# asmuth-archive/libsmatrix

Measured on NVIDIA B200. Metric: incr_mops_c2, higher is better.
Workload: dtype u32

## Files before the change

libsmatrix_b200/csrc/smx_host.c:

```c
#define _GNU_SOURCE
#include <cuda_runtime_api.h>
#include <pthread.h>
#include <stdarg.h>
#include <stdio.h>
#include <stdlib.h>
#include <string.h>
#include <time.h>
#include <errno.h>
#include <fcntl.h>
#include <sys/stat.h>
#include <sys/types.h>
#include <unistd.h>

#include "../../include/smatrix.h"
#include "../../include/smatrix_b200.h"
#include "../../include/smatrix_batch.h"
#include "smx_internal.h"

#define SMX_DIR_LOG_DEFAULT 20u
#define SMX_CHUNK_DEFAULT (1u << 26)
#define SMX_STAGE_MAX (1u << 23)
#define SMX_SEG_MIN ((size_t)64 << 20)
#define SMX_SEG_MAX ((size_t)16 << 30)
#define SMX_MAX_ROUNDS 128
// ... 262 lines not shown
}
static void scratch_free(smatrix_t* s, void* p) {
  if (p && !s->arena_bytes) cudaFree(p);
}

static void ensure_lists(smatrix_t* s, uint32_t n) {
  if (n <= s->list_cap) return;
  uint32_t cap = s->list_cap ? s->list_cap : 1024;
  while (cap < n) cap *= 2;
  if (cap > s->chunk_max) cap = s->chunk_max > n ? s->chunk_max : n;
  if (s->arena_bytes && cap < s->chunk_max) cap = s->chunk_max;
  if (s->list_cap) {
    CK(cudaStreamSynchronize(s->stream));
    scratch_free(s, s->defer[0]); scratch_free(s, s->defer[1]); scratch_free(s, s->lists.late);
    scratch_free(s, s->lists.grow); scratch_free(s, s->lists.t0rows); scratch_free(s, s->lists.plan);
    scratch_free(s, s->lists.big); scratch_free(s, s->lists.mid);
  }
  s->defer[0] = (uint32_t*)scratch_alloc(s, (size_t)cap * 4);
  s->defer[1] = (uint32_t*)scratch_alloc(s, (size_t)cap * 4);
  s->lists.late = (uint32_t*)scratch_alloc(s, (size_t)cap * 4);
  s->lists.grow = (uint32_t*)scratch_alloc(s, (size_t)cap * 4);
  s->lists.t0rows = (uint32_t*)scratch_alloc(s, (size_t)cap * 4);
  s->lists.plan = (smx_plan_t*)scratch_alloc(s, (size_t)cap * sizeof(smx_plan_t));
  s->lists.big = (uint32_t*)scratch_alloc(s, (size_t)cap * 4);
  s->lists.mid = (uint32_t*)scratch_alloc(s, (size_t)cap * 4);
  s->list_cap = cap;
}

static void ensure_stage(smatrix_t* s, uint32_t n) {
  if (n <= s->stage_cap) return;
  uint32_t cap = n < 4096 ? 4096 : n;
  if (s->arena_bytes && cap < s->stage_max) cap = s->stage_max;
  if (s->stage_cap) {
    CK(cudaStreamSynchronize(s->stream));
    CK(cudaStreamSynchronize(s->copy_stream));
    for (int b = 0; b < 2; b++)
      for (int a = 0; a < 3; a++) scratch_free(s, s->stage[b][a]);
  }
  for (int b = 0; b < 2; b++)
    for (int a = 0; a < 3; a++) s->stage[b][a] = (uint32_t*)scratch_alloc(s, (size_t)cap * 4);
// ... 28 lines not shown
    if (have) CK(cudaMemcpyAsync(nb, s->free_ptr[c], (size_t)have * 8, cudaMemcpyDeviceToDevice, s->stream));
    s->free_ptr[c] = nb;
    copy_h2d(s, &s->d_ctl->free_stack[c], &s->free_ptr[c], sizeof nb, s->stream);
    s->free_cap[c] = (uint32_t)cap;
  }
}

static void grow_rows(smatrix_t* s, uint32_t n_grow) {
  smx_view_t v = view_of(s);
  double t0 = now_ns();
  smx_launch_grow_plan(s->stream, v, s->lists, n_grow);
  s->n_launches++;
  read_ctl(s);
  double t1 = now_ns();
  const size_t bytes = (size_t)s->h_ctl->plan_bytes;
  const uint32_t n_big = s->h_ctl->n_big, n_mid = s->h_ctl->n_mid;
  char* region = bytes ? slab_reserve(s, bytes) : NULL;
  s->bucket_bytes += bytes;
  if (s->recycle) {
    ensure_free_stacks(s);
    smx_launch_free_push(s->stream, v, s->lists, n_grow);
    s->n_launches++;
  }
  double t2 = now_ns();
  if (bytes && s->h_ctl->need_zero) CK(cudaMemsetAsync(region, 0, bytes, s->stream));
  const int tiles = s->migrate_tiles && n_big;
  smx_launch_migrate(s->stream, v, s->lists, n_grow, n_mid, n_big, region, tiles);
  if (tiles) {
    unsigned long long* spill;
    uint32_t n_spill;
    for (;;) {
      spill = dbuf_need(s, &s->db.spill, (size_t)s->spill_cap * 16);
      CK(cudaMemsetAsync(&s->d_ctl->n_spill, 0, 4, s->stream));
      smx_launch_migrate_tiles(s->stream, v, s->lists, n_big, region, spill, s->spill_cap);
      copy_d2h(s, &s->h_small->n_spill, &s->d_ctl->n_spill, 4, s->stream);
      CK(cudaStreamSynchronize(s->stream));
      n_spill = s->h_small->n_spill;
      if (n_spill <= s->spill_cap) break;
      s->spill_cap = n_spill + n_spill / 2 + 1024;
    }
    smx_launch_migrate_tiles_finish(s->stream, v, s->lists, n_big, region, spill, n_spill);
    s->n_spilled += n_spill;
  }
  if (s->timing) CK(cudaStreamSynchronize(s->stream));
  s->n_launches += (n_grow > n_mid + n_big ? 1 : 0) + (n_mid ? 1 : 0) + (n_big ? 3 : 0);
  s->n_row_grows += n_grow;
  s->n_recycled += s->h_ctl->n_recycled;
  s->phase_ns[PH_GROW_PLAN] += t1 - t0;
  s->phase_ns[PH_SLAB] += t2 - t1;
  s->phase_ns[PH_MIGRATE] += now_ns() - t2;
}

static double ln_unit(double r) {
  int k = 0;
  while (r < 0.5) { r *= 2.0; k++; }
  const double y = (r - 1.0) / (r + 1.0), y2 = y * y;
  double term = y, sum = 0.0;
  for (int i = 1; i < 40; i += 2) { sum += term / (double)i; term *= y2; }
  return 2.0 * sum - (double)k * 0.69314718055994530942;
}
// ... 1151 lines not shown
  if (s->fname && snapshot_save(s) != 0) {
    printf("libsmatrix error: could not write %s; the previous snapshot (if any) was kept\n", s->fname);
    fflush(stdout);
  }
  for (int i = 0; i < s->nsegs; i++)
    if (s->segs[i].owned) cudaFree(s->segs[i].base);
  free(s->segs);
  if (!s->dir_in_arena) cudaFree(s->dir);
  cudaFree(s->d_ctl);
  cudaFreeHost(s->h_ctl);
  cudaFree(s->d_small);
  cudaFreeHost(s->h_small);
  if (s->list_cap) {
    scratch_free(s, s->defer[0]); scratch_free(s, s->defer[1]); scratch_free(s, s->lists.late);
    scratch_free(s, s->lists.grow); scratch_free(s, s->lists.t0rows); scratch_free(s, s->lists.plan);
    scratch_free(s, s->lists.big); scratch_free(s, s->lists.mid);
  }
  scratch_free(s, s->addrs);
  if (s->part_cap)
    for (int a = 0; a < 4; a++) scratch_free(s, s->part[a]);
  if (s->stage_cap)
    for (int b = 0; b < 2; b++)
      for (int a = 0; a < 3; a++) scratch_free(s, s->stage[b][a]);
  const smx_dbuf_t* db = (const smx_dbuf_t*)&s->db;
  for (size_t b = 0; b < sizeof s->db / sizeof *db; b++) cudaFree(db[b].p);
  cudaEventDestroy(s->stage_ready[0]); cudaEventDestroy(s->stage_ready[1]);
  cudaEventDestroy(s->ev0); cudaEventDestroy(s->ev1);
  cudaEventDestroy(s->t_start); cudaEventDestroy(s->t_stop);
  cudaStreamDestroy(s->stream);
  cudaStreamDestroy(s->copy_stream);
  cudaStreamDestroy(s->read_stream[0]); cudaStreamDestroy(s->read_stream[1]);
// ... 93 lines not shown
      break;
    case SMX_STAT_RECYCLED: r = s->n_recycled; break;
    case SMX_STAT_BUCKET_BYTES: r = s->bucket_bytes; break;
    case SMX_STAT_SPILLED: r = s->n_spilled; break;
    case SMX_STAT_SLICED_GETS: r = s->n_sliced_gets; break;
    case SMX_STAT_WIDE_CHUNKS: r = s->n_wide_chunks; break;
    case SMX_STAT_NS_ALLOC: r = (uint64_t)s->alloc_ns; break;
    case SMX_STAT_ALLOCS: r = s->n_allocs; break;
    case SMX_STAT_TOPK_BIG: r = s->n_topk_big; break;
    case SMX_STAT_TOPK_PASSES: r = s->n_topk_passes; break;
    case SMX_STAT_H2D_BYTES: r = s->h2d_bytes; break;
    case SMX_STAT_D2H_BYTES: r = s->d2h_bytes; break;
    case SMX_STAT_DIR_CAP: r = s->dir_cap; break;
    case SMX_STAT_SLAB_BYTES: r = s->slab_bytes; break;
    case SMX_STAT_DEVICE_BYTES: {
      r = s->seg_bytes + s->dir_cap * sizeof(smx_row_t) + (uint64_t)s->list_cap * (6 * 4 + sizeof(smx_plan_t)) +
          (uint64_t)s->stage_cap * 24 + (uint64_t)s->addrs_cap * 8 + (uint64_t)s->part_cap * 16;
      const smx_dbuf_t* db = (const smx_dbuf_t*)&s->db;
      for (size_t b = 0; b < sizeof s->db / sizeof *db; b++) r += db[b].bytes;
      break;
    }
    case SMX_STAT_LAUNCHES: r = s->n_launches; break;
    case SMX_STAT_ROUNDS: r = s->n_rounds; break;
    case SMX_STAT_ROW_GROWS: r = s->n_row_grows; break;
    case SMX_STAT_DIR_GROWS: r = s->n_dir_grows; break;
    case SMX_STAT_KERNEL_NS: r = (uint64_t)s->kernel_ns; break;
    case SMX_STAT_NS_PARTITION: r = (uint64_t)s->phase_ns[PH_PARTITION]; break;
    case SMX_STAT_NS_UPSERT: r = (uint64_t)s->phase_ns[PH_UPSERT]; break;
    case SMX_STAT_NS_GROW_PLAN: r = (uint64_t)s->phase_ns[PH_GROW_PLAN]; break;
    case SMX_STAT_NS_SLAB: r = (uint64_t)s->phase_ns[PH_SLAB]; break;
    case SMX_STAT_NS_MIGRATE: r = (uint64_t)s->phase_ns[PH_MIGRATE]; break;
// ... 322 lines not shown
```

libsmatrix_b200/csrc/smx_internal.h:

```cpp
#ifndef SMX_INTERNAL_H
#define SMX_INTERNAL_H

#include <stddef.h>
#include <stdint.h>

#ifdef __cplusplus
extern "C" {
#endif

#define SMX_META_CAPLOG 0x3Fu
#define SMX_META_USED   0x100u
#define SMX_META_ZC     0x200u
#define SMX_META_D      0x400u
#define SMX_META_SLOG_SHIFT 16
#define SMX_META_SLOG   (0x1Fu << SMX_META_SLOG_SHIFT)
#define SMX_META_T0P    0x800u
#define SMX_META_GROW   0x1000u
#define SMX_INLINE_LOG  2u
#define SMX_MIN_SLAB_LOG 4u
#define SMX_MAX_CAPLOG  31u
#define SMX_BIG_LOG     13u
#define SMX_MID_LOG     9u
#define SMX_ZERO_LOG    9u
#define SMX_CLASSES     32u
#define SMX_PLAN_RECYCLED (1ull << 63)

typedef struct {
  uint32_t key;
  uint32_t meta;
  uint64_t slots;
  uint32_t live;
  uint32_t c0;
  uint32_t t0inv;
  uint32_t want;
  uint64_t inl[4];
} smx_row_t;

#define SMX_DIR_SLICES 256u
#define SMX_DIR_CREATE_STEPS 256u
typedef struct {
  unsigned long long dir_used;
  uint32_t n_late;
  uint32_t n_t0;
  uint32_t n_defer;
  uint32_t n_dirfull;
  uint32_t n_grow;
  uint32_t n_big;
  uint32_t n_mid;
  uint32_t n_recycled;
  uint32_t n_spill;
  uint32_t dir_probe_max;
  unsigned long long plan_bytes;
  unsigned long long need_zero;
  uint32_t grow_from[SMX_CLASSES];
  unsigned long long scratch;
  int32_t free_cnt[SMX_CLASSES];
  unsigned long long* free_stack[SMX_CLASSES];
  uint32_t slice_used[SMX_DIR_SLICES];
} smx_ctl_t;

typedef struct {
  smx_row_t* dir;
  uint64_t dir_cap;
  uint32_t slice_shift;
  uint32_t slice_limit;
  smx_ctl_t* ctl;
} smx_view_t;

typedef struct {
  const uint32_t* xs;
  const uint32_t* ys;
  const uint32_t* vs;
  const uint32_t* idx;
  uint32_t v_const;
  uint32_t n;
} smx_ops_t;

typedef struct {
  uint32_t entry;
  uint32_t newlog;
  uint64_t off;
} smx_plan_t;

typedef struct {
  uint32_t* defer_out;
  uint32_t* late;
  uint32_t* grow;
  uint32_t* t0rows;
  smx_plan_t* plan;
  uint32_t* big;
  uint32_t* mid;
} smx_lists_t;

enum { SMX_OP_INCR = 0, SMX_OP_DECR = 1, SMX_OP_SETZERO = 2 };
enum { SMX_PASS_COL0 = 0, SMX_PASS_EARLY = 1, SMX_PASS_LATE = 2 };

typedef void* smx_stream_t;

void smx_launch_upsert(smx_stream_t stream, smx_view_t v, smx_ops_t ops, smx_lists_t l, int op,
                       int pass, const uint32_t* list, uint32_t m, int preaggregate);
void smx_launch_grow_plan(smx_stream_t stream, smx_view_t v, smx_lists_t l, uint32_t n_grow);
void smx_launch_free_push(smx_stream_t stream, smx_view_t v, smx_lists_t l, uint32_t n_grow);
void smx_launch_migrate(smx_stream_t stream, smx_view_t v, smx_lists_t l, uint32_t n_grow,
                        uint32_t n_mid, uint32_t n_big, void* region_base, int skip_big);
void smx_launch_migrate_tiles(smx_stream_t stream, smx_view_t v, smx_lists_t l, uint32_t n_big, void* region_base,
                              unsigned long long* spill, uint32_t spill_cap);
void smx_launch_migrate_tiles_finish(smx_stream_t stream, smx_view_t v, smx_lists_t l, uint32_t n_big, void* region_base,
                                     const unsigned long long* spill, uint32_t n_spill);
void smx_launch_sketch(smx_stream_t stream, const uint32_t* xs, uint32_t n, uint32_t* bitmap,
                       uint32_t bits_log, smx_ctl_t* ctl);
void smx_launch_live_bytes(smx_stream_t stream, smx_view_t v);
void smx_launch_dir_rehash(smx_stream_t stream, smx_view_t from, smx_view_t to);
void smx_launch_finalize_t0(smx_stream_t stream, smx_view_t v, const uint32_t* t0rows, uint32_t n);
void smx_launch_sync_rowlen(smx_stream_t stream, smx_view_t v, const uint32_t* rows, uint32_t n);
void smx_launch_set_max(smx_stream_t stream, smx_view_t v, smx_ops_t ops, uint64_t* addrs);
void smx_launch_set_commit(smx_stream_t stream, smx_ops_t ops, uint64_t* addrs);
size_t smx_batch_out_sort_bytes(uint32_t n);
void smx_launch_batch_out(smx_stream_t stream, smx_view_t v, smx_ops_t ops, int op, uint32_t* out,
                          uint64_t* addrs_a, uint64_t* addrs_b, uint32_t* idx_a, uint32_t* idx_b,
// ... 96 lines not shown
```

libsmatrix_b200/csrc/smx_kernels.cu:

```cuda
#include "smx_internal.h"

#ifdef SMX_HOSTSIM
#include "hostsim.h"
#include "cuda_runtime_api.h"
#include <algorithm>
#include <vector>
#else
#include <cuda_runtime.h>
#include <cub/device/device_radix_sort.cuh>
#define SMX_WARP 32
#define SMX_LAUNCH(kern, grid, block, stream, ...) \
  kern<<<(grid), (block), 0, (cudaStream_t)(stream)>>>(__VA_ARGS__)
#define SMX_ACTIVEMASK(key) __activemask()
#endif

typedef unsigned long long ull;
#define SMX_FULL 0xffffffffu
#if defined(SMX_HOSTSIM) && SMX_WARP == 1
#define SMX_BLOCK 1
#else
#define SMX_BLOCK (8 * SMX_WARP)
#endif

#define SCAN_PER_THREAD 8
// ... 69 lines not shown
  h.t0inv = (uint32_t)c[3];
  h.want = (uint32_t)(c[3] >> 32);
  return h;
}

__device__ __forceinline__ uint32_t lane_id() { return threadIdx.x % SMX_WARP; }

__device__ __forceinline__ uint32_t agg_inc(uint32_t* ctr) {
  unsigned m = SMX_ACTIVEMASK(ctr);
  uint32_t lane = lane_id();
  int leader = __ffs(m) - 1;
  uint32_t base = 0;
  if ((int)lane == leader) base = atomicAdd(ctr, (uint32_t)__popc(m));
  base = __shfl_sync(m, base, leader);
  return base + (uint32_t)__popc(m & ((1u << lane) - 1u));
}
__device__ __forceinline__ void agg_inc64(ull* ctr) {
  unsigned m = SMX_ACTIVEMASK(ctr);
  if ((int)lane_id() == __ffs(m) - 1) atomicAdd(ctr, (ull)__popc(m));
}

__host__ __device__ __forceinline__ uint32_t rowlen_catch_up(uint32_t meta, uint32_t live, bool z) {
  uint32_t slog = 4u + ((meta & SMX_META_SLOG) >> SMX_META_SLOG_SHIFT);
  uint32_t d = (meta & SMX_META_D) ? 1u : 0u;
  if (live) {
    const ull last = (ull)live - 1u;
    while (slog < 36u && last + d > (1ull << (slog - 1u))) {
      ++slog;
      d = z ? 1u : d;
    }
  }
  return (meta & ~(SMX_META_SLOG | SMX_META_D)) | ((slog - 4u) << SMX_META_SLOG_SHIFT) | (d ? SMX_META_D : 0u);
}

// ... 218 lines not shown
  __syncthreads();
  const uint32_t nd = s_ndefer < 4u * SMX_BLOCK ? s_ndefer : 4u * SMX_BLOCK;
  if (threadIdx.x == 0 && nd) {
    s_base = atomicAdd(&V.ctl->n_defer, nd);
    if (s_ndirfull) atomicAdd(&V.ctl->n_dirfull, s_ndirfull);
  }
  __syncthreads();
  for (uint32_t k = threadIdx.x; k < nd; k += blockDim.x) S.defer_out[s_base + k] = s_defer[k];
}

#define SMX_SMEM_MIGRATE_LOG 8u
#define SMX_MID_SMEM_LOG 12u

__global__ void __launch_bounds__(SMX_BLOCK)
k_grow_plan(smx_view_t V, smx_lists_t S, uint32_t n_grow) {
  const uint32_t lane = lane_id();
  const uint32_t stride = gridDim.x * blockDim.x;
  const uint32_t n_up = (n_grow + (SMX_WARP - 1)) / SMX_WARP * SMX_WARP;
  for (uint32_t j = blockIdx.x * blockDim.x + threadIdx.x; j < n_up; j += stride) {
    const bool act = j < n_grow;
    ull bytes = 0, recycled = 0;
    uint32_t entry = 0, newlog = 0, caplog = 0;
    if (act) {
      entry = S.grow[j];
      Hdr h = ld_hdr(V.dir + entry);
      caplog = h.meta & SMX_META_CAPLOG;
      const ull need = 2ull * ((ull)h.live + (ull)h.want);
      newlog = caplog + (caplog < 8u ? 3u : (caplog >= SMX_MID_LOG ? 2u : 1u));
      if (newlog > 8u && caplog < 8u) newlog = 8u;
      if (newlog < SMX_MIN_SLAB_LOG) newlog = SMX_MIN_SLAB_LOG;
      while ((1ull << newlog) < need && newlog < SMX_MAX_CAPLOG) ++newlog;
      {
        const unsigned grp = __match_any_sync(SMX_ACTIVEMASK(0), newlog);
        const int leader = __ffs(grp) - 1;
        const int cnt = __popc(grp), rank = __popc(grp & ((1u << lane) - 1u));
        int base = 0;
        if ((int)lane == leader) {
          base = atomicSub(&V.ctl->free_cnt[newlog], cnt);
          if (base < cnt) atomicAdd(&V.ctl->free_cnt[newlog], cnt - (base > 0 ? base : 0));
        }
        base = __shfl_sync(grp, base, leader);
        const int at = base - 1 - rank;
        if (at >= 0) recycled = (ull)V.ctl->free_stack[newlog][at];
      }
      bytes = recycled ? 0ull : (8ull << newlog);
      if (caplog > SMX_INLINE_LOG) {
        const unsigned grp = __match_any_sync(SMX_ACTIVEMASK(0), caplog);
        if ((int)lane == __ffs(grp) - 1) atomicAdd(&V.ctl->grow_from[caplog], (uint32_t)__popc(grp));
      }
    }
    ull incl = bytes;
    for (uint32_t d = 1; d < SMX_WARP; d <<= 1) {
      ull t = __shfl_up_sync(SMX_FULL, incl, d);
      if (lane >= d) incl += t;
    }
    const ull total = __shfl_sync(SMX_FULL, incl, SMX_WARP - 1);
    ull base = 0;
    if (lane == 0 && total) base = atomicAdd(&V.ctl->plan_bytes, total);
    base = __shfl_sync(SMX_FULL, base, 0);
    if (act) {
      smx_plan_t p;
      p.entry = entry;
      p.newlog = newlog;
      p.off = recycled ? (SMX_PLAN_RECYCLED | recycled) : (base + incl - bytes);
      S.plan[j] = p;
      if (recycled) agg_inc(&V.ctl->n_recycled);
      const bool by_grid = caplog >= SMX_BIG_LOG || (caplog >= SMX_MID_LOG && newlog > SMX_MID_SMEM_LOG);
      if (by_grid) S.big[agg_inc(&V.ctl->n_big)] = j;
      else if (caplog >= SMX_MID_LOG) S.mid[agg_inc(&V.ctl->n_mid)] = j;
      const bool in_place = by_grid || (caplog < SMX_MID_LOG && newlog > SMX_SMEM_MIGRATE_LOG);
      if (in_place && !recycled) agg_inc64(&V.ctl->need_zero);
    }
  }
}

__global__ void __launch_bounds__(SMX_BLOCK)
k_free_push(smx_view_t V, smx_lists_t S, uint32_t n_grow) {
  const uint32_t lane = lane_id();
  for (uint32_t j = blockIdx.x * blockDim.x + threadIdx.x; j < n_grow; j += gridDim.x * blockDim.x) {
    const Hdr h = ld_hdr(V.dir + S.plan[j].entry);
    const uint32_t caplog = h.meta & SMX_META_CAPLOG;
    if (caplog <= SMX_INLINE_LOG) continue;
    const unsigned grp = __match_any_sync(SMX_ACTIVEMASK(0), caplog);
    const int leader = __ffs(grp) - 1;
    int base = 0;
    if ((int)lane == leader) base = atomicAdd(&V.ctl->free_cnt[caplog], __popc(grp));
    base = __shfl_sync(grp, base, leader);
    V.ctl->free_stack[caplog][base + __popc(grp & ((1u << lane) - 1u))] = h.slots;
  }
}

__device__ __forceinline__ void place_cell(ull* base, uint32_t caplog, ull cell) {
  const uint32_t nsec = 1u << (caplog - 2u);
  uint32_t s = smx_mix_col((uint32_t)cell) & (nsec - 1u);
  for (uint32_t probe = 0; probe < nsec; ++probe, s = (s + 1u) & (nsec - 1u)) {
    ull* sec = base + 4ull * s;
    ull c[4];
    ld_sector(sec, c);
#pragma unroll
    for (int k = 0; k < 4; ++k) {
      if (c[k] != 0ull) continue;
      if (atomicCAS(sec + k, 0ull, cell) == 0ull) return;
    }
  }
}
__device__ __forceinline__ void place_cell_smem(ull* sb, uint32_t nsec, ull c) {
  uint32_t sidx = smx_mix_col((uint32_t)c) & (nsec - 1u);
  for (bool placed = false; !placed; sidx = (sidx + 1u) & (nsec - 1u))
    for (int k = 0; k < 4 && !placed; ++k)
      placed = (atomicCAS(&sb[4u * sidx + k], 0ull, c) == 0ull);
}

__device__ __forceinline__ ull* plan_bucket(const smx_plan_t& p, char* region) {
  return (p.off & SMX_PLAN_RECYCLED) ? (ull*)(p.off & ~SMX_PLAN_RECYCLED) : (ull*)(region + p.off);
}

__device__ __forceinline__ void finish_growth(smx_row_t* e, const Hdr& h, ull* nb, uint32_t newlog) {
  e->slots = (ull)nb;
  e->want = 0u;
  e->meta = (h.meta & ~(SMX_META_CAPLOG | SMX_META_GROW)) | newlog;
}

__global__ void __launch_bounds__(SMX_BLOCK)
k_migrate(smx_view_t V, smx_lists_t S, uint32_t n_grow, char* region) {
  __shared__ ull sbuf[SMX_BLOCK / SMX_WARP][1u << SMX_SMEM_MIGRATE_LOG];
  const uint32_t lane = lane_id();
  const uint32_t wib = threadIdx.x / SMX_WARP;
  const uint32_t warp = (blockIdx.x * blockDim.x + threadIdx.x) / SMX_WARP;
  const uint32_t nwarps = gridDim.x * blockDim.x / SMX_WARP;
  for (uint32_t j = warp; j < n_grow; j += nwarps) {
    const smx_plan_t p = S.plan[j];
    smx_row_t* e = V.dir + p.entry;
    const Hdr h = ld_hdr(e);
    const uint32_t caplog = h.meta & SMX_META_CAPLOG;
    if (caplog >= SMX_MID_LOG) continue;
    ull* ob = (caplog == SMX_INLINE_LOG) ? (ull*)e->inl : (ull*)h.slots;
    ull* nb = plan_bucket(p, region);
    const uint32_t cap = 1u << caplog;
    if (p.newlog <= SMX_SMEM_MIGRATE_LOG) {
      ull* sb = sbuf[wib];
      const uint32_t ncap = 1u << p.newlog, nsec = ncap >> 2;
      for (uint32_t i = lane; i < ncap; i += SMX_WARP) sb[i] = 0ull;
      __syncwarp();
      for (uint32_t s0 = lane; s0 < cap; s0 += SMX_WARP) {
        const ull c = ob[s0];
        if (c != 0ull) place_cell_smem(sb, nsec, c);
      }
      __syncwarp();
      for (uint32_t i = lane; i < ncap; i += SMX_WARP) nb[i] = sb[i];
    } else {
      for (uint32_t s0 = lane; s0 < cap; s0 += SMX_WARP) {
        const ull c = ob[s0];
        if (c != 0ull) place_cell(nb, p.newlog, c);
      }
    }
    __syncwarp();
    if (lane == 0) finish_growth(e, h, nb, p.newlog);
  }
}

__global__ void __launch_bounds__(SMX_BLOCK)
k_migrate_mid(smx_view_t V, smx_lists_t S, uint32_t n_mid, char* region) {
  __shared__ ull sb[1u << SMX_MID_SMEM_LOG];
  for (uint32_t j = blockIdx.x; j < n_mid; j += gridDim.x) {
    const smx_plan_t p = S.plan[S.mid[j]];
    smx_row_t* e = V.dir + p.entry;
    const Hdr h = ld_hdr(e);
    const uint32_t caplog = h.meta & SMX_META_CAPLOG;
    ull* ob = (ull*)h.slots;
    ull* nb = plan_bucket(p, region);
    const uint32_t cap = 1u << caplog;
    {
      const uint32_t ncap = 1u << p.newlog, nsec = ncap >> 2;
      for (uint32_t i = threadIdx.x; i < ncap; i += blockDim.x) sb[i] = 0ull;
      __syncthreads();
      for (uint32_t s0 = threadIdx.x; s0 < cap; s0 += blockDim.x) {
        const ull c = ob[s0];
        ob[s0] = 0ull;
        if (c != 0ull) place_cell_smem(sb, nsec, c);
      }
      __syncthreads();
      for (uint32_t i = threadIdx.x; i < ncap; i += blockDim.x) nb[i] = sb[i];
    }
    __syncthreads();
    if (threadIdx.x == 0) finish_growth(e, h, nb, p.newlog);
    __syncthreads();
  }
}

__global__ void __launch_bounds__(SMX_BLOCK)
k_migrate_big(smx_view_t V, smx_lists_t S, uint32_t big_first, char* region) {
  const smx_plan_t p = S.plan[S.big[big_first + blockIdx.y]];
  smx_row_t* e = V.dir + p.entry;
  const Hdr h = ld_hdr(e);
  const uint32_t caplog = h.meta & SMX_META_CAPLOG;
  ull* ob = (ull*)h.slots;
  ull* nb = plan_bucket(p, region);
  const ull cap = 1ull << caplog;
  for (ull s = blockIdx.x * blockDim.x + threadIdx.x; s < cap; s += (ull)gridDim.x * blockDim.x) {
    const ull c = ob[s];
    ob[s] = 0ull;
    if (c != 0ull) place_cell(nb, p.newlog, c);
  }
}
__global__ void k_migrate_big_finish(smx_view_t V, smx_lists_t S, uint32_t n_big, char* region) {
  for (uint32_t b = blockIdx.x * blockDim.x + threadIdx.x; b < n_big; b += gridDim.x * blockDim.x) {
    const smx_plan_t p = S.plan[S.big[b]];
    smx_row_t* e = V.dir + p.entry;
    const Hdr h = ld_hdr(e);
    finish_growth(e, h, plan_bucket(p, region), p.newlog);
  }
}

#ifndef MIG_TILE_LOG
#define MIG_TILE_LOG 10u
#endif
#define MIG_TILE (1u << MIG_TILE_LOG)
__device__ __forceinline__ bool sector_is_full(const ull* sec) {
  ull c[4];
  ld_sector(sec, c);
  return c[0] != 0ull && c[1] != 0ull && c[2] != 0ull && c[3] != 0ull;
}
__device__ __forceinline__ void tile_take_sector(const ull* sec, ull* sm, uint32_t t0, uint32_t n_new, uint32_t j,
                                                 smx_ctl_t* ctl, ull* spill, uint32_t spill_cap) {
  ull c[4];
// ... 6 lines not shown
    bool placed = false;
    for (uint32_t q = hn - t0; q < MIG_TILE && !placed; ++q)
      for (int w = 0; w < 4 && !placed; ++w) placed = (atomicCAS(&sm[4u * q + w], 0ull, c[k]) == 0ull);
    if (!placed) {
      const uint32_t at = atomicAdd(&ctl->n_spill, 1u);
      if (at < spill_cap) { spill[2ull * at] = (ull)j; spill[2ull * at + 1] = c[k]; }
    }
  }
}
__global__ void __launch_bounds__(SMX_BLOCK)
k_migrate_tiles(smx_view_t V, smx_lists_t S, uint32_t big_first, char* region, ull* spill, uint32_t spill_cap) {
  __shared__ ull sm[4u * MIG_TILE];
  __shared__ uint32_t s_stop;
  const uint32_t j = S.big[big_first + blockIdx.y];
  const smx_plan_t p = S.plan[j];
  const smx_row_t* e = V.dir + p.entry;
  const Hdr h = ld_hdr(e);
  const ull* ob = (const ull*)h.slots;
  ull* nb = plan_bucket(p, region);
  const uint32_t n_old = 1u << ((h.meta & SMX_META_CAPLOG) - 2u), n_new = 1u << (p.newlog - 2u);
  const uint32_t n_tiles = n_new >> MIG_TILE_LOG, mask = n_old - 1u;
  const uint32_t len = n_old < MIG_TILE ? n_old : MIG_TILE;
  for (uint32_t t = blockIdx.x; t < n_tiles; t += gridDim.x) {
    const uint32_t t0 = t << MIG_TILE_LOG;
    const uint32_t r0 = n_old < MIG_TILE ? 0u : (t0 & mask);
    for (uint32_t i = threadIdx.x; i < 4u * MIG_TILE; i += blockDim.x) sm[i] = 0ull;
    __syncthreads();
    for (uint32_t s = threadIdx.x; s < len; s += blockDim.x)
      tile_take_sector(ob + 4ull * ((r0 + s) & mask), sm, t0, n_new, j, V.ctl, spill, spill_cap);
    if (len < n_old) {
      for (uint32_t base = len, step = SMX_WARP; base < n_old; base += step, step = blockDim.x) {
        if (threadIdx.x == 0) s_stop = 0xFFFFFFFFu;
        __syncthreads();
        const uint32_t s = base + threadIdx.x;
        const bool in = threadIdx.x < step && s < n_old;
// ... 3 lines not shown
        if (in && s < stop) tile_take_sector(ob + 4ull * ((r0 + s) & mask), sm, t0, n_new, j, V.ctl, spill, spill_cap);
        __syncthreads();
        if (stop != 0xFFFFFFFFu) break;
      }
    }
    __syncthreads();
    ull* out = nb + 4ull * t0;
    for (uint32_t i = threadIdx.x; i < 4u * MIG_TILE; i += blockDim.x) out[i] = sm[i];
    __syncthreads();
  }
}
__global__ void __launch_bounds__(SMX_BLOCK)
k_spill_insert(smx_view_t V, smx_lists_t S, char* region, const ull* spill, uint32_t n_spill) {
  for (uint32_t i = blockIdx.x * blockDim.x + threadIdx.x; i < n_spill; i += gridDim.x * blockDim.x) {
    const smx_plan_t p = S.plan[(uint32_t)spill[2ull * i]];
    place_cell(plan_bucket(p, region), p.newlog, spill[2ull * i + 1]);
  }
}
__global__ void __launch_bounds__(SMX_BLOCK)
k_zero_old_big(smx_view_t V, smx_lists_t S, uint32_t big_first) {
  const smx_plan_t p = S.plan[S.big[big_first + blockIdx.y]];
  const Hdr h = ld_hdr(V.dir + p.entry);
  ull* ob = (ull*)h.slots;
  const ull cap = 1ull << (h.meta & SMX_META_CAPLOG);
  for (ull s = blockIdx.x * (ull)blockDim.x + threadIdx.x; s < cap; s += (ull)gridDim.x * blockDim.x) ob[s] = 0ull;
}

__global__ void __launch_bounds__(SMX_BLOCK) k_dir_rehash(smx_view_t from, smx_view_t to) {
  const ull mask = to.dir_cap - 1;
  uint32_t far = 0;
  for (ull pos = blockIdx.x * blockDim.x + threadIdx.x; pos < from.dir_cap;
       pos += (ull)gridDim.x * blockDim.x) {
    const smx_row_t* o = from.dir + pos;
    ull a[4], b[4];
    ld_hsector(o, a);
    if (!((a[0] >> 32) & SMX_META_USED)) continue;
    ld_hsector((const char*)o + 32, b);
    const ull home = smx_mix_row((uint32_t)a[0]) & mask;
    for (ull step = 0;; ++step) {
// ... 1271 lines not shown
    auto k = k_upsert<SMX_OP_SETZERO>;
    SMX_LAUNCH(k, grid, SMX_BLOCK, st, v, ops, l, pass, list, m, pre);
  }
}

extern "C" void smx_launch_grow_plan(smx_stream_t st, smx_view_t v, smx_lists_t l, uint32_t n_grow) {
  if (!n_grow) return;
  SMX_LAUNCH(k_grow_plan, grid_for(n_grow), SMX_BLOCK, st, v, l, n_grow);
}

extern "C" void smx_launch_free_push(smx_stream_t st, smx_view_t v, smx_lists_t l, uint32_t n_grow) {
  if (!n_grow) return;
  SMX_LAUNCH(k_free_push, grid_for(n_grow), SMX_BLOCK, st, v, l, n_grow);
}

extern "C" void smx_launch_migrate(smx_stream_t st, smx_view_t v, smx_lists_t l, uint32_t n_grow,
                                   uint32_t n_mid, uint32_t n_big, void* region, int skip_big) {
  if (!n_grow) return;
  if (n_grow > n_mid + n_big)
    SMX_LAUNCH(k_migrate, grid_for((ull)n_grow * SMX_WARP), SMX_BLOCK, st, v, l, n_grow, (char*)region);
  if (n_mid) {
    const uint32_t cap = (uint32_t)smx_grid_blocks();
    SMX_LAUNCH(k_migrate_mid, n_mid < cap ? n_mid : cap, SMX_BLOCK, st, v, l, n_mid, (char*)region);
  }
  if (skip_big) return;
  for (uint32_t first = 0; first < n_big; first += 32768u) {
    const uint32_t cnt = (n_big - first < 32768u) ? n_big - first : 32768u;
    dim3 grid(SMX_WARP > 1 ? 64u : 2u, cnt, 1u);
    SMX_LAUNCH(k_migrate_big, grid, SMX_BLOCK, st, v, l, first, (char*)region);
  }
  if (n_big) SMX_LAUNCH(k_migrate_big_finish, grid_for(n_big), SMX_BLOCK, st, v, l, n_big, (char*)region);
}

extern "C" void smx_launch_migrate_tiles(smx_stream_t st, smx_view_t v, smx_lists_t l, uint32_t n_big, void* region,
                                         unsigned long long* spill, uint32_t spill_cap) {
// ... 386 lines not shown
```

Baseline: 13260.

## Restructure row-growth planning and warp migration with block aggregation and prefetch

The grow-plan kernel now gathers its counters (plan bytes, big/mid/wide list counts, recycled, grow_from, need_zero) in shared memory per block and issues one global atomic per block, where before each warp hit the global counters directly. Each plan now records the old slot pointer and meta, so the migration kernels no longer reread directory headers. Warp migration is templated by shared-memory size, adds a separate pass for rows growing to 2^9 slots, loads each row's old cells into registers while the previous row is being placed, and copies with 16-byte accesses. Old mid buckets are zeroed only above a raised threshold, and the migrate grid is capped at resident occupancy. In exchange the plan struct is larger, the kernel adds block barriers, and the free-count check ahead of recycling reads a value that other threads change concurrently.

```diff
diff --git a/libsmatrix_b200/csrc/smx_host.c b/libsmatrix_b200/csrc/smx_host.c
--- a/libsmatrix_b200/csrc/smx_host.c
+++ b/libsmatrix_b200/csrc/smx_host.c
@@ -300,7 +300,7 @@
     CK(cudaStreamSynchronize(s->stream));
     scratch_free(s, s->defer[0]); scratch_free(s, s->defer[1]); scratch_free(s, s->lists.late);
     scratch_free(s, s->lists.grow); scratch_free(s, s->lists.t0rows); scratch_free(s, s->lists.plan);
-    scratch_free(s, s->lists.big); scratch_free(s, s->lists.mid);
+    scratch_free(s, s->lists.big); scratch_free(s, s->lists.mid); scratch_free(s, s->lists.wide);
   }
   s->defer[0] = (uint32_t*)scratch_alloc(s, (size_t)cap * 4);
   s->defer[1] = (uint32_t*)scratch_alloc(s, (size_t)cap * 4);
@@ -310,6 +310,7 @@
   s->lists.plan = (smx_plan_t*)scratch_alloc(s, (size_t)cap * sizeof(smx_plan_t));
   s->lists.big = (uint32_t*)scratch_alloc(s, (size_t)cap * 4);
   s->lists.mid = (uint32_t*)scratch_alloc(s, (size_t)cap * 4);
+  s->lists.wide = (uint32_t*)scratch_alloc(s, (size_t)cap * 4);
   s->list_cap = cap;
 }
 
@@ -368,7 +369,7 @@
   read_ctl(s);
   double t1 = now_ns();
   const size_t bytes = (size_t)s->h_ctl->plan_bytes;
-  const uint32_t n_big = s->h_ctl->n_big, n_mid = s->h_ctl->n_mid;
+  const uint32_t n_big = s->h_ctl->n_big, n_mid = s->h_ctl->n_mid, n_wide = s->h_ctl->n_wide;
   char* region = bytes ? slab_reserve(s, bytes) : NULL;
   s->bucket_bytes += bytes;
   if (s->recycle) {
@@ -379,7 +380,7 @@
   double t2 = now_ns();
   if (bytes && s->h_ctl->need_zero) CK(cudaMemsetAsync(region, 0, bytes, s->stream));
   const int tiles = s->migrate_tiles && n_big;
-  smx_launch_migrate(s->stream, v, s->lists, n_grow, n_mid, n_big, region, tiles);
+  smx_launch_migrate(s->stream, v, s->lists, n_grow, n_mid, n_big, n_wide, region, tiles);
   if (tiles) {
     unsigned long long* spill;
     uint32_t n_spill;
@@ -397,7 +398,7 @@
     s->n_spilled += n_spill;
   }
   if (s->timing) CK(cudaStreamSynchronize(s->stream));
-  s->n_launches += (n_grow > n_mid + n_big ? 1 : 0) + (n_mid ? 1 : 0) + (n_big ? 3 : 0);
+  s->n_launches += (n_grow > n_mid + n_big + n_wide ? 1 : 0) + (n_wide ? 1 : 0) + (n_mid ? 1 : 0) + (n_big ? 3 : 0);
   s->n_row_grows += n_grow;
   s->n_recycled += s->h_ctl->n_recycled;
   s->phase_ns[PH_GROW_PLAN] += t1 - t0;
@@ -1579,7 +1580,7 @@
   if (s->list_cap) {
     scratch_free(s, s->defer[0]); scratch_free(s, s->defer[1]); scratch_free(s, s->lists.late);
     scratch_free(s, s->lists.grow); scratch_free(s, s->lists.t0rows); scratch_free(s, s->lists.plan);
-    scratch_free(s, s->lists.big); scratch_free(s, s->lists.mid);
+    scratch_free(s, s->lists.big); scratch_free(s, s->lists.mid); scratch_free(s, s->lists.wide);
   }
   scratch_free(s, s->addrs);
   if (s->part_cap)
@@ -1703,7 +1704,7 @@
     case SMX_STAT_DIR_CAP: r = s->dir_cap; break;
     case SMX_STAT_SLAB_BYTES: r = s->slab_bytes; break;
     case SMX_STAT_DEVICE_BYTES: {
-      r = s->seg_bytes + s->dir_cap * sizeof(smx_row_t) + (uint64_t)s->list_cap * (6 * 4 + sizeof(smx_plan_t)) +
+      r = s->seg_bytes + s->dir_cap * sizeof(smx_row_t) + (uint64_t)s->list_cap * (7 * 4 + sizeof(smx_plan_t)) +
           (uint64_t)s->stage_cap * 24 + (uint64_t)s->addrs_cap * 8 + (uint64_t)s->part_cap * 16;
       const smx_dbuf_t* db = (const smx_dbuf_t*)&s->db;
       for (size_t b = 0; b < sizeof s->db / sizeof *db; b++) r += db[b].bytes;
diff --git a/libsmatrix_b200/csrc/smx_internal.h b/libsmatrix_b200/csrc/smx_internal.h
--- a/libsmatrix_b200/csrc/smx_internal.h
+++ b/libsmatrix_b200/csrc/smx_internal.h
@@ -21,7 +21,8 @@
 #define SMX_MAX_CAPLOG  31u
 #define SMX_BIG_LOG     13u
 #define SMX_MID_LOG     9u
-#define SMX_ZERO_LOG    9u
+#define SMX_WIDE_LOG    9u
+#define SMX_ZERO_LOG    10u
 #define SMX_CLASSES     32u
 #define SMX_PLAN_RECYCLED (1ull << 63)
 
@@ -51,7 +52,8 @@
   uint32_t n_spill;
   uint32_t dir_probe_max;
   unsigned long long plan_bytes;
-  unsigned long long need_zero;
+  uint32_t need_zero;
+  uint32_t n_wide;
   uint32_t grow_from[SMX_CLASSES];
   unsigned long long scratch;
   int32_t free_cnt[SMX_CLASSES];
@@ -80,6 +82,9 @@
   uint32_t entry;
   uint32_t newlog;
   uint64_t off;
+  uint64_t old;
+  uint32_t meta;
+  uint32_t pad;
 } smx_plan_t;
 
 typedef struct {
@@ -90,6 +95,7 @@
   smx_plan_t* plan;
   uint32_t* big;
   uint32_t* mid;
+  uint32_t* wide;
 } smx_lists_t;
 
 enum { SMX_OP_INCR = 0, SMX_OP_DECR = 1, SMX_OP_SETZERO = 2 };
@@ -102,7 +108,7 @@
 void smx_launch_grow_plan(smx_stream_t stream, smx_view_t v, smx_lists_t l, uint32_t n_grow);
 void smx_launch_free_push(smx_stream_t stream, smx_view_t v, smx_lists_t l, uint32_t n_grow);
 void smx_launch_migrate(smx_stream_t stream, smx_view_t v, smx_lists_t l, uint32_t n_grow,
-                        uint32_t n_mid, uint32_t n_big, void* region_base, int skip_big);
+                        uint32_t n_mid, uint32_t n_big, uint32_t n_wide, void* region_base, int skip_big);
 void smx_launch_migrate_tiles(smx_stream_t stream, smx_view_t v, smx_lists_t l, uint32_t n_big, void* region_base,
                               unsigned long long* spill, uint32_t spill_cap);
 void smx_launch_migrate_tiles_finish(smx_stream_t stream, smx_view_t v, smx_lists_t l, uint32_t n_big, void* region_base,
diff --git a/libsmatrix_b200/csrc/smx_kernels.cu b/libsmatrix_b200/csrc/smx_kernels.cu
--- a/libsmatrix_b200/csrc/smx_kernels.cu
+++ b/libsmatrix_b200/csrc/smx_kernels.cu
@@ -107,10 +107,6 @@
   if ((int)lane == leader) base = atomicAdd(ctr, (uint32_t)__popc(m));
   base = __shfl_sync(m, base, leader);
   return base + (uint32_t)__popc(m & ((1u << lane) - 1u));
-}
-__device__ __forceinline__ void agg_inc64(ull* ctr) {
-  unsigned m = SMX_ACTIVEMASK(ctr);
-  if ((int)lane_id() == __ffs(m) - 1) atomicAdd(ctr, (ull)__popc(m));
 }
 
 __host__ __device__ __forceinline__ uint32_t rowlen_catch_up(uint32_t meta, uint32_t live, bool z) {
@@ -359,23 +355,37 @@
 
 __global__ void __launch_bounds__(SMX_BLOCK)
 k_grow_plan(smx_view_t V, smx_lists_t S, uint32_t n_grow) {
+  enum { C_BIG = 0, C_MID, C_WIDE, C_RECYCLED, C_N };
+  __shared__ ull s_bytes, s_bytes_base;
+  __shared__ uint32_t s_zero, s_cnt[C_N], s_base[C_N], s_from[SMX_CLASSES];
   const uint32_t lane = lane_id();
   const uint32_t stride = gridDim.x * blockDim.x;
-  const uint32_t n_up = (n_grow + (SMX_WARP - 1)) / SMX_WARP * SMX_WARP;
-  for (uint32_t j = blockIdx.x * blockDim.x + threadIdx.x; j < n_up; j += stride) {
+  for (uint32_t j0 = blockIdx.x * blockDim.x; j0 < n_grow; j0 += stride) {
+    const uint32_t j = j0 + threadIdx.x;
     const bool act = j < n_grow;
-    ull bytes = 0, recycled = 0;
-    uint32_t entry = 0, newlog = 0, caplog = 0;
+    if (threadIdx.x == 0) {
+      s_bytes = 0ull;
+      s_zero = 0u;
+      for (int k = 0; k < C_N; ++k) s_cnt[k] = 0u;
+    }
+    for (uint32_t c = threadIdx.x; c < SMX_CLASSES; c += blockDim.x) s_from[c] = 0u;
+    __syncthreads();
+    ull bytes = 0, recycled = 0, old = 0;
+    uint32_t entry = 0, newlog = 0, caplog = 0, meta = 0;
+    int list = -1;
+    uint32_t at_list = 0;
     if (act) {
       entry = S.grow[j];
-      Hdr h = ld_hdr(V.dir + entry);
+      const Hdr h = ld_hdr(V.dir + entry);
+      meta = h.meta;
       caplog = h.meta & SMX_META_CAPLOG;
+      old = caplog == SMX_INLINE_LOG ? (ull)V.dir[entry].inl : h.slots;
       const ull need = 2ull * ((ull)h.live + (ull)h.want);
       newlog = caplog + (caplog < 8u ? 3u : (caplog >= SMX_MID_LOG ? 2u : 1u));
       if (newlog > 8u && caplog < 8u) newlog = 8u;
       if (newlog < SMX_MIN_SLAB_LOG) newlog = SMX_MIN_SLAB_LOG;
       while ((1ull << newlog) < need && newlog < SMX_MAX_CAPLOG) ++newlog;
-      {
+      if (*(volatile int32_t*)&V.ctl->free_cnt[newlog] > 0) {
         const unsigned grp = __match_any_sync(SMX_ACTIVEMASK(0), newlog);
         const int leader = __ffs(grp) - 1;
         const int cnt = __popc(grp), rank = __popc(grp & ((1u << lane) - 1u));
@@ -391,8 +401,20 @@
       bytes = recycled ? 0ull : (8ull << newlog);
       if (caplog > SMX_INLINE_LOG) {
         const unsigned grp = __match_any_sync(SMX_ACTIVEMASK(0), caplog);
-        if ((int)lane == __ffs(grp) - 1) atomicAdd(&V.ctl->grow_from[caplog], (uint32_t)__popc(grp));
+        if ((int)lane == __ffs(grp) - 1) atomicAdd(&s_from[caplog], (uint32_t)__popc(grp));
       }
+      if (recycled) agg_inc(&s_cnt[C_RECYCLED]);
+      const bool by_grid = caplog >= SMX_BIG_LOG || (caplog >= SMX_MID_LOG && newlog > SMX_MID_SMEM_LOG);
+      list = by_grid ? C_BIG : caplog >= SMX_MID_LOG ? C_MID : newlog == SMX_WIDE_LOG ? C_WIDE : -1;
+      if (list >= 0) {
+        const unsigned grp = __match_any_sync(SMX_ACTIVEMASK(0), list);
+        const int leader = __ffs(grp) - 1;
+        uint32_t base = 0;
+        if ((int)lane == leader) base = atomicAdd(&s_cnt[list], (uint32_t)__popc(grp));
+        at_list = __shfl_sync(grp, base, leader) + (uint32_t)__popc(grp & ((1u << lane) - 1u));
+      }
+      const bool in_place = by_grid || (caplog < SMX_MID_LOG && newlog > SMX_WIDE_LOG);
+      if (in_place && !recycled) agg_inc(&s_zero);
     }
     ull incl = bytes;
     for (uint32_t d = 1; d < SMX_WARP; d <<= 1) {
@@ -400,21 +422,31 @@
       if (lane >= d) incl += t;
     }
     const ull total = __shfl_sync(SMX_FULL, incl, SMX_WARP - 1);
-    ull base = 0;
-    if (lane == 0 && total) base = atomicAdd(&V.ctl->plan_bytes, total);
-    base = __shfl_sync(SMX_FULL, base, 0);
+    ull wbase = 0;
+    if (lane == 0 && total) wbase = atomicAdd(&s_bytes, total);
+    wbase = __shfl_sync(SMX_FULL, wbase, 0);
+    __syncthreads();
+    if (threadIdx.x == 0) {
+      s_bytes_base = s_bytes ? atomicAdd(&V.ctl->plan_bytes, s_bytes) : 0ull;
+      if (s_zero) atomicAdd(&V.ctl->need_zero, s_zero);
+      if (s_cnt[C_BIG]) s_base[C_BIG] = atomicAdd(&V.ctl->n_big, s_cnt[C_BIG]);
+      if (s_cnt[C_MID]) s_base[C_MID] = atomicAdd(&V.ctl->n_mid, s_cnt[C_MID]);
+      if (s_cnt[C_WIDE]) s_base[C_WIDE] = atomicAdd(&V.ctl->n_wide, s_cnt[C_WIDE]);
+      if (s_cnt[C_RECYCLED]) atomicAdd(&V.ctl->n_recycled, s_cnt[C_RECYCLED]);
+    }
+    for (uint32_t c = threadIdx.x; c < SMX_CLASSES; c += blockDim.x)
+      if (s_from[c]) atomicAdd(&V.ctl->grow_from[c], s_from[c]);
+    __syncthreads();
     if (act) {
       smx_plan_t p;
       p.entry = entry;
       p.newlog = newlog;
-      p.off = recycled ? (SMX_PLAN_RECYCLED | recycled) : (base + incl - bytes);
+      p.off = recycled ? (SMX_PLAN_RECYCLED | recycled) : (s_bytes_base + wbase + incl - bytes);
+      p.old = old;
+      p.meta = meta;
+      p.pad = 0u;
       S.plan[j] = p;
-      if (recycled) agg_inc(&V.ctl->n_recycled);
-      const bool by_grid = caplog >= SMX_BIG_LOG || (caplog >= SMX_MID_LOG && newlog > SMX_MID_SMEM_LOG);
-      if (by_grid) S.big[agg_inc(&V.ctl->n_big)] = j;
-      else if (caplog >= SMX_MID_LOG) S.mid[agg_inc(&V.ctl->n_mid)] = j;
-      const bool in_place = by_grid || (caplog < SMX_MID_LOG && newlog > SMX_SMEM_MIGRATE_LOG);
-      if (in_place && !recycled) agg_inc64(&V.ctl->need_zero);
+      if (list >= 0) (list == C_BIG ? S.big : list == C_MID ? S.mid : S.wide)[s_base[list] + at_list] = j;
     }
   }
 }
@@ -423,15 +455,15 @@
 k_free_push(smx_view_t V, smx_lists_t S, uint32_t n_grow) {
   const uint32_t lane = lane_id();
   for (uint32_t j = blockIdx.x * blockDim.x + threadIdx.x; j < n_grow; j += gridDim.x * blockDim.x) {
-    const Hdr h = ld_hdr(V.dir + S.plan[j].entry);
-    const uint32_t caplog = h.meta & SMX_META_CAPLOG;
+    const smx_plan_t p = S.plan[j];
+    const uint32_t caplog = p.meta & SMX_META_CAPLOG;
     if (caplog <= SMX_INLINE_LOG) continue;
     const unsigned grp = __match_any_sync(SMX_ACTIVEMASK(0), caplog);
     const int leader = __ffs(grp) - 1;
     int base = 0;
     if ((int)lane == leader) base = atomicAdd(&V.ctl->free_cnt[caplog], __popc(grp));
     base = __shfl_sync(grp, base, leader);
-    V.ctl->free_stack[caplog][base + __popc(grp & ((1u << lane) - 1u))] = h.slots;
+    V.ctl->free_stack[caplog][base + __popc(grp & ((1u << lane) - 1u))] = p.old;
   }
 }
 
@@ -456,51 +488,104 @@
       placed = (atomicCAS(&sb[4u * sidx + k], 0ull, c) == 0ull);
 }
 
-__device__ __forceinline__ ull* plan_bucket(const smx_plan_t& p, char* region) {
-  return (p.off & SMX_PLAN_RECYCLED) ? (ull*)(p.off & ~SMX_PLAN_RECYCLED) : (ull*)(region + p.off);
-}
-
-__device__ __forceinline__ void finish_growth(smx_row_t* e, const Hdr& h, ull* nb, uint32_t newlog) {
+__device__ __forceinline__ ull* plan_bucket(ull off, char* region) {
+  return (off & SMX_PLAN_RECYCLED) ? (ull*)(off & ~SMX_PLAN_RECYCLED) : (ull*)(region + off);
+}
+
+__device__ __forceinline__ void finish_growth(smx_row_t* e, uint32_t meta, ull* nb, uint32_t newlog) {
   e->slots = (ull)nb;
   e->want = 0u;
-  e->meta = (h.meta & ~(SMX_META_CAPLOG | SMX_META_GROW)) | newlog;
-}
-
-__global__ void __launch_bounds__(SMX_BLOCK)
-k_migrate(smx_view_t V, smx_lists_t S, uint32_t n_grow, char* region) {
-  __shared__ ull sbuf[SMX_BLOCK / SMX_WARP][1u << SMX_SMEM_MIGRATE_LOG];
+  e->meta = (meta & ~(SMX_META_CAPLOG | SMX_META_GROW)) | newlog;
+}
+
+__device__ __forceinline__ void copy16(ull* dst, const ull* src) {
+#ifdef SMX_HOSTSIM
+  dst[0] = src[0];
+  dst[1] = src[1];
+#else
+  *(ulonglong2*)dst = *(const ulonglong2*)src;
+#endif
+}
+__device__ __forceinline__ void zero16(ull* p) {
+#ifdef SMX_HOSTSIM
+  p[0] = 0ull;
+  p[1] = 0ull;
+#else
+  *(ulonglong2*)p = make_ulonglong2(0ull, 0ull);
+#endif
+}
+
+__device__ __forceinline__ uint32_t plan_u32(uint32_t v, int src) { return __shfl_sync(SMX_FULL, v, src); }
+__device__ __forceinline__ ull plan_u64(ull v, int src) { return __shfl_sync(SMX_FULL, v, src); }
+template <uint32_t K>
+__device__ __forceinline__ void mig_fetch(const smx_plan_t& mine, int r, uint32_t lane, ull c[K]) {
+  const uint32_t cap = 1u << (plan_u32(mine.meta, r) & SMX_META_CAPLOG);
+  const ull* ob = (const ull*)plan_u64(mine.old, r);
+#pragma unroll
+  for (uint32_t k = 0; k < K; ++k) c[k] = lane + k * SMX_WARP < cap ? ob[lane + k * SMX_WARP] : 0ull;
+}
+template <uint32_t SLOG, uint32_t K>
+__device__ __forceinline__ void mig_build(const smx_view_t& V, const smx_plan_t& mine, int r, const ull c[K], ull* sb,
+                                          uint32_t lane, char* region) {
+  const uint32_t newlog = plan_u32(mine.newlog, r), meta = plan_u32(mine.meta, r);
+  ull* nb = plan_bucket(plan_u64(mine.off, r), region);
+  if (newlog <= SLOG) {
+    const uint32_t ncap = 1u << newlog, nsec = ncap >> 2;
+    for (uint32_t i = 2u * lane; i < ncap; i += 2u * SMX_WARP) zero16(sb + i);
+    __syncwarp();
+#pragma unroll
+    for (uint32_t k = 0; k < K; ++k)
+      if (c[k] != 0ull) place_cell_smem(sb, nsec, c[k]);
+    __syncwarp();
+    for (uint32_t i = 2u * lane; i < ncap; i += 2u * SMX_WARP) copy16(nb + i, sb + i);
+  } else {
+    const ull* ob = (const ull*)plan_u64(mine.old, r);
+    const uint32_t cap = 1u << (meta & SMX_META_CAPLOG);
+    for (uint32_t s0 = lane; s0 < cap; s0 += SMX_WARP)
+      if (ob[s0] != 0ull) place_cell(nb, newlog, ob[s0]);
+  }
+  const uint32_t entry = plan_u32(mine.entry, r);
+  __syncwarp();
+  if (lane == 0) finish_growth(V.dir + entry, meta, nb, newlog);
+}
+
+template <uint32_t SLOG>
+__global__ void __launch_bounds__(SMX_BLOCK)
+k_migrate(smx_view_t V, smx_lists_t S, const uint32_t* list, uint32_t n, char* region) {
+  constexpr uint32_t K = (1u << (SLOG - 1u)) / SMX_WARP;
+  alignas(16) __shared__ ull sbuf[SMX_BLOCK / SMX_WARP][1u << SLOG];
+  ull* const sb = sbuf[threadIdx.x / SMX_WARP];
   const uint32_t lane = lane_id();
-  const uint32_t wib = threadIdx.x / SMX_WARP;
   const uint32_t warp = (blockIdx.x * blockDim.x + threadIdx.x) / SMX_WARP;
-  const uint32_t nwarps = gridDim.x * blockDim.x / SMX_WARP;
-  for (uint32_t j = warp; j < n_grow; j += nwarps) {
-    const smx_plan_t p = S.plan[j];
-    smx_row_t* e = V.dir + p.entry;
-    const Hdr h = ld_hdr(e);
-    const uint32_t caplog = h.meta & SMX_META_CAPLOG;
-    if (caplog >= SMX_MID_LOG) continue;
-    ull* ob = (caplog == SMX_INLINE_LOG) ? (ull*)e->inl : (ull*)h.slots;
-    ull* nb = plan_bucket(p, region);
-    const uint32_t cap = 1u << caplog;
-    if (p.newlog <= SMX_SMEM_MIGRATE_LOG) {
-      ull* sb = sbuf[wib];
-      const uint32_t ncap = 1u << p.newlog, nsec = ncap >> 2;
-      for (uint32_t i = lane; i < ncap; i += SMX_WARP) sb[i] = 0ull;
-      __syncwarp();
-      for (uint32_t s0 = lane; s0 < cap; s0 += SMX_WARP) {
-        const ull c = ob[s0];
-        if (c != 0ull) place_cell_smem(sb, nsec, c);
+  const ull nwarps = gridDim.x * blockDim.x / SMX_WARP;
+  for (ull b = warp; b < n; b += SMX_WARP * nwarps) {
+    const ull jl = b + lane * nwarps;
+    smx_plan_t mine = {};
+    bool take = false;
+    if (jl < n) {
+      mine = S.plan[list ? list[jl] : (uint32_t)jl];
+      const uint32_t caplog = mine.meta & SMX_META_CAPLOG;
+      take = list != nullptr || (caplog < SMX_MID_LOG && mine.newlog != SMX_WIDE_LOG);
+    }
+    unsigned todo = __ballot_sync(SMX_FULL, take);
+    if (!todo) continue;
+    int cur = __ffs(todo) - 1;
+    todo &= todo - 1u;
+    ull c[K];
+    mig_fetch<K>(mine, cur, lane, c);
+    for (;;) {
+      const int nxt = todo ? __ffs(todo) - 1 : -1;
+      ull cn[K];
+      if (nxt >= 0) {
+        todo &= todo - 1u;
+        mig_fetch<K>(mine, nxt, lane, cn);
       }
-      __syncwarp();
-      for (uint32_t i = lane; i < ncap; i += SMX_WARP) nb[i] = sb[i];
-    } else {
-      for (uint32_t s0 = lane; s0 < cap; s0 += SMX_WARP) {
-        const ull c = ob[s0];
-        if (c != 0ull) place_cell(nb, p.newlog, c);
-      }
-    }
-    __syncwarp();
-    if (lane == 0) finish_growth(e, h, nb, p.newlog);
+      mig_build<SLOG, K>(V, mine, cur, c, sb, lane, region);
+      if (nxt < 0) break;
+      cur = nxt;
+#pragma unroll
+      for (uint32_t k = 0; k < K; ++k) c[k] = cn[k];
+    }
   }
 }
 
@@ -509,26 +594,25 @@
   __shared__ ull sb[1u << SMX_MID_SMEM_LOG];
   for (uint32_t j = blockIdx.x; j < n_mid; j += gridDim.x) {
     const smx_plan_t p = S.plan[S.mid[j]];
-    smx_row_t* e = V.dir + p.entry;
-    const Hdr h = ld_hdr(e);
-    const uint32_t caplog = h.meta & SMX_META_CAPLOG;
-    ull* ob = (ull*)h.slots;
-    ull* nb = plan_bucket(p, region);
+    const uint32_t caplog = p.meta & SMX_META_CAPLOG;
+    ull* ob = (ull*)p.old;
+    ull* nb = plan_bucket(p.off, region);
     const uint32_t cap = 1u << caplog;
+    const bool zero_old = caplog >= SMX_ZERO_LOG;
     {
       const uint32_t ncap = 1u << p.newlog, nsec = ncap >> 2;
       for (uint32_t i = threadIdx.x; i < ncap; i += blockDim.x) sb[i] = 0ull;
       __syncthreads();
       for (uint32_t s0 = threadIdx.x; s0 < cap; s0 += blockDim.x) {
         const ull c = ob[s0];
-        ob[s0] = 0ull;
+        if (zero_old) ob[s0] = 0ull;
         if (c != 0ull) place_cell_smem(sb, nsec, c);
       }
       __syncthreads();
       for (uint32_t i = threadIdx.x; i < ncap; i += blockDim.x) nb[i] = sb[i];
     }
     __syncthreads();
-    if (threadIdx.x == 0) finish_growth(e, h, nb, p.newlog);
+    if (threadIdx.x == 0) finish_growth(V.dir + p.entry, p.meta, nb, p.newlog);
     __syncthreads();
   }
 }
@@ -536,12 +620,9 @@
 __global__ void __launch_bounds__(SMX_BLOCK)
 k_migrate_big(smx_view_t V, smx_lists_t S, uint32_t big_first, char* region) {
   const smx_plan_t p = S.plan[S.big[big_first + blockIdx.y]];
-  smx_row_t* e = V.dir + p.entry;
-  const Hdr h = ld_hdr(e);
-  const uint32_t caplog = h.meta & SMX_META_CAPLOG;
-  ull* ob = (ull*)h.slots;
-  ull* nb = plan_bucket(p, region);
-  const ull cap = 1ull << caplog;
+  ull* ob = (ull*)p.old;
+  ull* nb = plan_bucket(p.off, region);
+  const ull cap = 1ull << (p.meta & SMX_META_CAPLOG);
   for (ull s = blockIdx.x * blockDim.x + threadIdx.x; s < cap; s += (ull)gridDim.x * blockDim.x) {
     const ull c = ob[s];
     ob[s] = 0ull;
@@ -551,9 +632,7 @@
 __global__ void k_migrate_big_finish(smx_view_t V, smx_lists_t S, uint32_t n_big, char* region) {
   for (uint32_t b = blockIdx.x * blockDim.x + threadIdx.x; b < n_big; b += gridDim.x * blockDim.x) {
     const smx_plan_t p = S.plan[S.big[b]];
-    smx_row_t* e = V.dir + p.entry;
-    const Hdr h = ld_hdr(e);
-    finish_growth(e, h, plan_bucket(p, region), p.newlog);
+    finish_growth(V.dir + p.entry, p.meta, plan_bucket(p.off, region), p.newlog);
   }
 }
 
@@ -590,11 +669,9 @@
   __shared__ uint32_t s_stop;
   const uint32_t j = S.big[big_first + blockIdx.y];
   const smx_plan_t p = S.plan[j];
-  const smx_row_t* e = V.dir + p.entry;
-  const Hdr h = ld_hdr(e);
-  const ull* ob = (const ull*)h.slots;
-  ull* nb = plan_bucket(p, region);
-  const uint32_t n_old = 1u << ((h.meta & SMX_META_CAPLOG) - 2u), n_new = 1u << (p.newlog - 2u);
+  const ull* ob = (const ull*)p.old;
+  ull* nb = plan_bucket(p.off, region);
+  const uint32_t n_old = 1u << ((p.meta & SMX_META_CAPLOG) - 2u), n_new = 1u << (p.newlog - 2u);
   const uint32_t n_tiles = n_new >> MIG_TILE_LOG, mask = n_old - 1u;
   const uint32_t len = n_old < MIG_TILE ? n_old : MIG_TILE;
   for (uint32_t t = blockIdx.x; t < n_tiles; t += gridDim.x) {
@@ -628,15 +705,14 @@
 k_spill_insert(smx_view_t V, smx_lists_t S, char* region, const ull* spill, uint32_t n_spill) {
   for (uint32_t i = blockIdx.x * blockDim.x + threadIdx.x; i < n_spill; i += gridDim.x * blockDim.x) {
     const smx_plan_t p = S.plan[(uint32_t)spill[2ull * i]];
-    place_cell(plan_bucket(p, region), p.newlog, spill[2ull * i + 1]);
+    place_cell(plan_bucket(p.off, region), p.newlog, spill[2ull * i + 1]);
   }
 }
 __global__ void __launch_bounds__(SMX_BLOCK)
 k_zero_old_big(smx_view_t V, smx_lists_t S, uint32_t big_first) {
   const smx_plan_t p = S.plan[S.big[big_first + blockIdx.y]];
-  const Hdr h = ld_hdr(V.dir + p.entry);
-  ull* ob = (ull*)h.slots;
-  const ull cap = 1ull << (h.meta & SMX_META_CAPLOG);
+  ull* ob = (ull*)p.old;
+  const ull cap = 1ull << (p.meta & SMX_META_CAPLOG);
   for (ull s = blockIdx.x * (ull)blockDim.x + threadIdx.x; s < cap; s += (ull)gridDim.x * blockDim.x) ob[s] = 0ull;
 }
 
@@ -1938,11 +2014,34 @@
   SMX_LAUNCH(k_free_push, grid_for(n_grow), SMX_BLOCK, st, v, l, n_grow);
 }
 
+template <class F>
+static uint32_t grid_resident(F kern, ull items) {
+  uint32_t g = grid_for(items);
+#ifndef SMX_HOSTSIM
+  int per_sm = 0;
+  if (cudaOccupancyMaxActiveBlocksPerMultiprocessor(&per_sm, kern, SMX_BLOCK, 0) == cudaSuccess && per_sm > 0) {
+    const uint32_t cap = (uint32_t)per_sm * (uint32_t)(smx_grid_blocks() / 8);
+    if (g > cap) g = cap;
+  }
+#else
+  (void)kern;
+#endif
+  return g;
+}
+
 extern "C" void smx_launch_migrate(smx_stream_t st, smx_view_t v, smx_lists_t l, uint32_t n_grow,
-                                   uint32_t n_mid, uint32_t n_big, void* region, int skip_big) {
+                                   uint32_t n_mid, uint32_t n_big, uint32_t n_wide, void* region, int skip_big) {
   if (!n_grow) return;
-  if (n_grow > n_mid + n_big)
-    SMX_LAUNCH(k_migrate, grid_for((ull)n_grow * SMX_WARP), SMX_BLOCK, st, v, l, n_grow, (char*)region);
+  if (n_grow > n_mid + n_big + n_wide) {
+    auto k = k_migrate<SMX_SMEM_MIGRATE_LOG>;
+    SMX_LAUNCH(k, grid_resident(k, (ull)n_grow * SMX_WARP), SMX_BLOCK, st, v, l, (const uint32_t*)nullptr, n_grow,
+               (char*)region);
+  }
+  if (n_wide) {
+    auto k = k_migrate<SMX_WIDE_LOG>;
+    SMX_LAUNCH(k, grid_resident(k, (ull)n_wide * SMX_WARP), SMX_BLOCK, st, v, l, (const uint32_t*)l.wide, n_wide,
+               (char*)region);
+  }
   if (n_mid) {
     const uint32_t cap = (uint32_t)smx_grid_blocks();
     SMX_LAUNCH(k_migrate_mid, n_mid < cap ? n_mid : cap, SMX_BLOCK, st, v, l, n_mid, (char*)region);
```

New measurement: 13630, median of 6. +2.8%, better.
